# mir-group/pair_allegro

Hardware: AMD Instinct MI355X
Metric: atom_steps_per_sec (higher is better)
Workload: dtype f32-equivalent (f16x2 split on the f16 matrix cores, f32 accumulate); 1 GPU; BASELINE config 4: 1000000-atom bulk Si (50^3 diamond cells), model S (l_max=1, U=32, S=64, 2 layers), r_max 5.0 A + skin 1.0 A, NVE dt=1 fs; grid=1x1x1, rebuilds=4, comm=serial, comm_transport=library/hosted/single-rank gather-scatter

## Files before the change

pair_allegro_amd/csrc/allegro_hip.hip:

```cpp
#include "../../include/allegro_hip.h"

#include <pthread.h>
#include <sched.h>

#include <algorithm>
#include <array>
#include <cmath>
#include <cstdio>
#include <cstdlib>
#include <cstring>
#include <atomic>
#include <condition_variable>
#include <functional>
#include <map>
#include <mutex>
#include <new>
#include <string>
#include <thread>
#include <vector>

#include "engine.h"
#include "generic_engine.h"

using namespace ahip;
// ... 274 lines not shown
    } else if (k == "cutoff_compare") {
      m->cutoff_strict = word("le|lt") == 1;
      m->h_cutsq_dev.clear();
    } else if (k == "edge_schedule") {
      m->opt_edge_schedule = (Model::EdgeSchedule)word(Model::EDGE_SCHEDULE_WORDS);
    } else if (k == "tile_pack") {
      m->opt_tile_pack = (Model::TilePack)word(Model::TILE_PACK_WORDS);
    } else if (k == "dense_centres") {
      m->opt_dense_centres = (Model::DenseCentres)word(Model::DENSE_CENTRES_WORDS);
    } else if (k == "wide_tile") {
      const Model::WideTile o = (Model::WideTile)word(Model::WIDE_TILE_WORDS);
      if (o != m->opt_wide_tile) { m->opt_wide_tile = o; fusedlx_free(*m); }
    } else if (k == "lx64_mlp_width") {
      const Model::Lx64MlpWidth o = (Model::Lx64MlpWidth)word(Model::LX64_MLP_WIDTH_WORDS);
      if (o != m->opt_lx64_mlp_width) { m->opt_lx64_mlp_width = o; fusedlx_free(*m); }
    } else if (k == "timing") {
      m->timing = (v == "1" || v == "on" || v == "true");
    } else throw ArgError("unknown option '" + k + "'");
  });
}

namespace ahip {
namespace {
struct Staging {
  std::mutex mu;
  void *p = nullptr;
  std::map<int, std::array<hipEvent_t, 2>> evs;
  hipEvent_t *ev = nullptr;
  static constexpr size_t BYTES = 8u << 20, HALF = BYTES / 2;
  void *get() {
// ... 1032 lines not shown
```

pair_allegro_amd/csrc/engine.h:

```cpp
#pragma once
#include <hip/hip_runtime.h>

#include <atomic>
#include <map>
#include <stdexcept>
#include <algorithm>
#include <cmath>
#include <cstdlib>
#include <string>
#include <vector>

#include "arith_policy.h"
#include "fused_shapes.h"
#include "model_io.h"
#include "prims.h"

namespace ahip {

struct HipError : std::runtime_error {
  explicit HipError(const std::string &m) : std::runtime_error(m) {}
};
struct ArgError : std::runtime_error {
  explicit ArgError(const std::string &m) : std::runtime_error(m) {}
};
// ... 72 lines not shown

  enum class Path { Auto, Fused, Generic };
  static constexpr const char *PATH_WORDS = "auto|fused|generic";
  enum class Precision { Model, Float64 };
  static constexpr const char *PRECISION_WORDS = "model|float64";
  enum class TilePack { Auto, Separate, Fused };
  static constexpr const char *TILE_PACK_WORDS = "auto|separate|fused";
  enum class EdgeSchedule { Auto, Static, Dynamic };
  static constexpr const char *EDGE_SCHEDULE_WORDS = "auto|static|dynamic";
  enum class DenseCentres { Whole, Split };
  static constexpr const char *DENSE_CENTRES_WORDS = "whole|split";
  enum class WideTile { S64, Auto };
  static constexpr const char *WIDE_TILE_WORDS = "64|auto";
  enum class Lx64MlpWidth { W64, Auto };
  static constexpr const char *LX64_MLP_WIDTH_WORDS = "64|auto";
  Path opt_path = Path::Auto;
  Precision opt_precision = Precision::Model;
  FusedTb opt_fused_tb = FusedTb::Table;
  ArithState arith;
  DevBuf b_chk;
  HostModel hm_fused;
  bool hm_fused_ready = false;
  std::vector<int> active;
  std::vector<int> active_set;
  std::vector<int> active_mapped;
  unsigned char *slot_dev = nullptr;
  const unsigned char *slot_cur = nullptr;
  std::vector<double> rcut_fused_host;
  double *rcut_fused_dev = nullptr;
  long long chunk_edges = 2000000;
  int reserve_wgs = 0;
  bool timing = false;
  TilePack opt_tile_pack = TilePack::Auto;
  EdgeSchedule opt_edge_schedule = EdgeSchedule::Auto;
  DenseCentres opt_dense_centres = DenseCentres::Whole;
  WideTile opt_wide_tile = WideTile::S64;
  Lx64MlpWidth opt_lx64_mlp_width = Lx64MlpWidth::W64;
  bool cutoff_strict = false;

  DeviceWeights<float> wf;
  DeviceWeights<double> wd;
  void *cg_dev = nullptr;
  int ncg_full = 0, ncg_scalar = 0;
  double *rcut_model_dev = nullptr;

  int inum = 0, nall = 0;
  long long nneigh = 0;
  bool have_list = false;
  int max_list_row = -1;
  const int *d_ilist = nullptr, *d_nloff = nullptr, *d_nlj = nullptr;
  DevBuf b_ilist, b_nloff, b_nlj;
  std::vector<int> h_flat_j, h_off32, h_ilist;
// ... 191 lines not shown
```

pair_allegro_amd/csrc/fused.hip:

```cpp
#include <hip/hip_runtime.h>

#include <cmath>
#include <algorithm>
#include <cstdio>
#include <cstdlib>
#include <cstring>
#include <type_traits>

#include "../../include/allegro_hip.h"
#include "engine.h"
#define AHIP_RING 4
#include "fused_common.h"
#include "fused_h.h"
#include "fused_rows.h"
#include "prims.h"

#ifndef AHIP_FUSED_PART
#define AHIP_FUSED_PART 0
#endif
namespace ahip {


[[maybe_unused]] static constexpr int MAX_TILE_SLOTS = 128;
static constexpr int MAXNL = 3;
// ... 15 lines not shown
  const int *maxdeg_sel;
  const float *wbase;
  int wbytes;
  int o_stream;
  int o_tbtab, tb_nk;
  int o_tpl, o_pair, o_out1, o_scale, o_shift;
  int o_res[MAXNL];
  float *scratch;
  long long wg_scratch, wave_scratch;
  double *f, *eatom, *partial;
  long long *prof;
  float *dbg;
  float cp[6];
  int *err;
  double *vatom;
};

template <int NW, int NL = MAXNL, int RT = 2> struct __attribute__((aligned(16))) Lds {
  static constexpr int SLOTS = 16 * NW;
  static constexpr int MAXA = NW == 4 ? 6 : 12;
  float stage[SLOTS * STG_LD];
  float env[NL][MAXA * ENV_LD];
  float denv[MAXA * ENV_LD];
  float tp[NL][5 * 32];
  float park[NW][8 * ROW];
  double eacc[MAXA];
  double virw[NW][6];
  int aoff[2][MAXA + 2];
  float rc[16];
  float scale[16], shift[16];
// ... 124 lines not shown
      acc3 += lds.stage[(sl + 3) * STG_LD + fidx];
    }
    for (; sl < s1; ++sl) acc0 += lds.stage[sl * STG_LD + fidx];
    dst[a * ENV_LD + fidx] = scale * ((acc0 + acc1) + (acc2 + acc3));
  }
}
enum { PH_GEOM = 0, PH_TB, PH_EMB, PH_ENV, PH_TP, PH_MIX, PH_LAT, PH_OUT, PH_BLAT, PH_BMIX, PH_BTP, PH_BENV, PH_BEMB, PH_BTB, PH_FIN, PH_N };
#define PHASE(id) do { if (PROF) { long long _t = clock64(); pacc[id] += _t - tprev; tprev = _t; } } while (0)

template <int AR> struct RingT {
  int act = 1;
  f32x4 f[AR != 0 ? 1 : RING];
  u32x4 b[AR == 0 ? 1 : (AR == 1 ? RINGB : AR == 2 ? RINGB2 : RINGH)];
};
template <int AR, int KT, int NT, bool ACC, int RPI, bool BR = true, class Epi>
__device__ __forceinline__ void lin(__amdgpu_buffer_rsrc_t W, int &wp, const f32x4 (&in)[KT], f32x4 (&out)[NT], int v16, RingT<AR> &ring, Epi epi) {
  if (BR && !ring.act) {
    if constexpr (!ACC) {
#pragma unroll
      for (int t = 0; t < NT; ++t) out[t] = f32x4{0.f, 0.f, 0.f, 0.f};
    }
    return;
  }
  if constexpr (AR == 3) {
    static_assert(KT % 2 == 0, "K-steps are pairs of 16-feature tiles");
    Hop b[1][KT / 2], unused[1][NT / 2];
#pragma unroll
    for (int ks = 0; ks < KT / 2; ++ks) b[0][ks] = split_pair_h(in[2 * ks], in[2 * ks + 1]);
    Epi ep[1] = {epi};
    linear_h<1, KT / 2, NT, ACC, false, (4 * RPI) % RINGH, Epi, true>(W, wp, b, reinterpret_cast<f32x4 (&)[1][NT]>(out), unused, v16, ring.b, ep);
  } else if constexpr (AR != 0) {
    static_assert(KT % 2 == 0, "K-steps are pairs of 16-feature tiles");
    constexpr int NTERM = AR == 1 ? 3 : 2;
    Bop b[KT / 2], unused[NT / 2];
#pragma unroll
    for (int ks = 0; ks < KT / 2; ++ks) b[ks] = split_pair(in[2 * ks], in[2 * ks + 1]);
    linear_b<KT / 2, NT, ACC, false, (2 * NTERM * RPI) % RingB<NTERM>::N, Epi, NTERM>(W, wp, b, out, unused, v16, ring.b, epi);
  } else {
    linear_s<KT, NT, ACC, (4 * RPI) % RING, Epi>(W, wp, in, out, v16, ring.f, epi);
  }
}

template <int RPI, bool BR = true, class Epi>
__device__ __forceinline__ void lin_m3(__amdgpu_buffer_rsrc_t W, int &wp, const f32x4 (&in0)[2], const f32x4 (&in1)[2], const f32x4 (&in2)[2], f32x4 (&out)[3][2], int v16,
                                       RingT<3> &ring, Epi (&epi)[3]) {
  if (BR && !ring.act) {
#pragma unroll
    for (int q = 0; q < 3; ++q) { out[q][0] = f32x4{0.f, 0.f, 0.f, 0.f}; out[q][1] = f32x4{0.f, 0.f, 0.f, 0.f}; }
    return;
  }
  Hop b[3][1], unused[3][1];
  b[0][0] = split_pair_h(in0[0], in0[1]); b[1][0] = split_pair_h(in1[0], in1[1]); b[2][0] = split_pair_h(in2[0], in2[1]);
  linear_h<3, 1, 2, false, false, (4 * RPI) % RINGH, Epi, true>(W, wp, b, out, unused, v16, ring.b, epi);
}
template <class Epi0, class Epi3>
__device__ __forceinline__ void lin_mix(__amdgpu_buffer_rsrc_t W, int &wp, const f32x4 (&in0)[2], const f32x4 (&in1)[2], const f32x4 (&in2)[2], const f32x4 (&in3)[2], f32x4 (&out0)[2],
                                        f32x4 (&out)[3][2], int v16, RingT<3> &ring, Epi0 epi0, Epi3 (&epi)[3]) {
  if (!ring.act) {
    out0[0] = f32x4{0.f, 0.f, 0.f, 0.f}; out0[1] = f32x4{0.f, 0.f, 0.f, 0.f};
#pragma unroll
    for (int q = 0; q < 3; ++q) { out[q][0] = f32x4{0.f, 0.f, 0.f, 0.f}; out[q][1] = f32x4{0.f, 0.f, 0.f, 0.f}; }
    return;
  }
  lin<3, 2, 2, false, 0, false>(W, wp, in0, out0, v16, ring, epi0);
  lin_m3<1, false>(W, wp, in1, in2, in3, out, v16, ring, epi);
}

struct TileIn {
  int a0, a1, e0, e1;
  float rx, ry, rz;
  int eii, jat, tt;
  int eoff;
};
struct TileBounds { int a0, a1, e0, e1; };
typedef const __attribute__((address_space(4))) int *cint_p;
__device__ __forceinline__ TileBounds tile_bounds(const FusedArgs &A, int tile, int ntiles) {
  const int tc = max(min(tile, ntiles - 1), 0);
  const cint_p ta = (cint_p)(unsigned long long)A.tile_a0, te = (cint_p)(unsigned long long)A.tile_e0;
  TileBounds b = {ta[tc], ta[tc + 1], te[tc], te[tc + 1]};
  if (tile >= ntiles) b = TileBounds{0, 0, 0, 0};
// ... 50 lines not shown
    const int pth = (k % 160) / 32;
    if (RT != 2 && k >= (NLT - 1) * 160 + 64) continue;
    lds.tp[k / 160][k % 160] = Wb[A.o_tpl + k] * (pth == 1 ? C_P1 : pth == 4 ? C_P4 : 1.f);
  }
  const int ntiles = *A.ntiles;
  constexpr int NL = NLT;
  double acc_part = 0.0;
  long long pacc[PH_N];
  long long tprev = 0;
  const long long t_clk0 = clock64(), t_wall0 = wall_clock64();
  if (PROF) {
#pragma unroll
    for (int k = 0; k < PH_N; ++k) pacc[k] = 0;
    tprev = clock64();
  }
  float *const pk = lds.park[wave];
  RingT<AR> ring;
  int wp = A.o_stream;
  if constexpr (AR != 0) ring_prime_b(WB, wp, v16, ring.b);
  else ring_prime(WB, wp, v16, ring.f);
  if (tid < MAXA) lds.eacc[tid] = 0.0;
  if (lane < 6) lds.virw[wave][lane] = 0.0;
  if (A.T <= 4 && tid < A.T * A.T) lds.rc[tid] = (float)A.rcut[tid];
  if (tid < A.T) { lds.scale[tid] = Wb[A.o_scale + tid]; lds.shift[tid] = Wb[A.o_shift + tid]; }
  if (tid < 2 * A.NL) lds.res[tid >> 1][tid & 1] = Wb[A.o_res[tid >> 1] + (tid & 1)];
  if constexpr (RT == 2) { if (tid >= 64 && tid < 96) lds.wo1[tid - 64] = Wb[A.o_out1 + tid - 64]; }
  else { if (tid >= 64 && tid < 64 + 16 * RT) lds.wo1v()[tid - 64] = Wb[A.o_out1 + tid - 64]; }

  const int s = wave * 16 + j;
  float *const st = lds.stage + s * STG_LD;
  if (tid == 0) lds.chunk[0] = (int)atomicAdd(A.tile_counter, (unsigned)A.tchunk);
// ... 3 lines not shown

  TileIn nx_;
  tile_fetch(A, tile_bounds(A, cbase, ntiles), s, tid, nx_);
  asm volatile("" : "+v"(nx_.rx), "+v"(nx_.ry), "+v"(nx_.rz), "+v"(nx_.eii), "+v"(nx_.jat), "+v"(nx_.tt), "+v"(nx_.eoff));

  for (;;) {
    const int tile = cbase + ck;
    if (tile >= ntiles) break;
    int claimed = 0;
    if (ck == 0 && tid == 0) {
      unsigned long long tcnt = (unsigned long long)A.tile_counter;
      asm volatile("" : "+v"(tcnt));
      claimed = (int)__hip_atomic_fetch_add((__attribute__((address_space(1))) unsigned int *)tcnt, (unsigned)A.tchunk, __ATOMIC_RELAXED, __HIP_MEMORY_SCOPE_AGENT);
    }
    const int a0 = nx_.a0, a1 = nx_.a1, e0 = nx_.e0, e1 = nx_.e1;
    const int wact = __builtin_amdgcn_readfirstlane(e0 + wave * 16 < e1 ? 1 : 0);
    ring.act = wact;
    const int v16t = wact ? v16 : 0x7ffffff0;
    const int na = a1 - a0;
    par ^= 1;
    int *const aoffp = lds.aoff[par];
    const int e = e0 + s;
    const bool valid = e < e1;
    const float rx = valid ? nx_.rx : 1.f, ry = nx_.ry, rz = nx_.rz;
    const int aloc = valid ? nx_.eii - a0 : 0, jat = nx_.jat, ti = nx_.tt >> 4, tj = nx_.tt & 15;
    if (tid <= na) aoffp[tid] = nx_.eoff - e0;
    const float d = sqrtf(rx * rx + ry * ry + rz * rz);
    const float inv = 1.f / d;
    const float nx = rx * inv, ny = ry * inv, nz = rz * inv;
    const float rc = A.T <= 4 ? lds.rc[ti * A.T + tj] : (float)A.rcut[ti * A.T + tj];
    const float xx = d / rc;
    float fc, dfc_dx;
    cutoff_poly_c(A.p, A.cp, xx, fc, dfc_dx);
    if (!valid) { fc = 0.f; dfc_dx = 0.f; }
// ... 2 lines not shown
    const float PI = 3.14159265358979323846f;
    const float *const envrow = lds.env[0] + aloc * ENV_LD;
    const float *const denvrow = lds.denv + aloc * ENV_LD;
    PHASE(PH_GEOM);

    f32x4 x[4];
    float tb_t = 0.f, tb_invh = 0.f;
    if constexpr (TBT) {
      tb_invh = (float)A.tb_nk / rc;
      const float sft = d * tb_invh;
      const int kq = min((int)sft, A.tb_nk - 1);
      tb_t = sft - (float)kq;
#ifdef ABL_NOTBGATHER
      const int tb_off = (A.o_tbtab + 4 * g) * 4;
#else
      const int tb_off = (A.o_tbtab + ((ti * A.T + tj) * A.tb_nk + kq) * 256 + 4 * g) * 4;
#endif
      const float vm = (valid && xx < 1.f) ? 1.f : 0.f;
#pragma unroll
      for (int t = 0; t < 4; ++t) {
        const f32x4 c0 = bload_w(WB, tb_off + (t * 4 + 0) * 64, 0), c1 = bload_w(WB, tb_off + (t * 4 + 1) * 64, 0);
        const f32x4 c2 = bload_w(WB, tb_off + (t * 4 + 2) * 64, 0), c3 = bload_w(WB, tb_off + (t * 4 + 3) * 64, 0);
        x[t] = (c0 + tb_t * (c1 + tb_t * (c2 + tb_t * c3))) * vm;
        bstore(SB, v16t, (R_Z1TB() + t) * ROW * 4, (c1 + tb_t * (2.f * c2 + (3.f * tb_t) * c3)) * (vm * tb_invh));
      }
    } else {
      f32x4 z[4], z2[4];
      {
        const float *pt = Wb + A.o_pair + (size_t)(ti * A.T + tj) * 64;
#pragma unroll
        for (int t = 0; t < 4; ++t) z[t] = *(const f32x4 *)(pt + 16 * t + 4 * g);
// ... 173 lines not shown
    eps = gsum(eps);
    asm volatile("" : "+v"(eps));

    float bsc = 1.f;
    if constexpr (AR == 3) {
      int bex;
      (void)frexpf(lds.scale[ti] * A.cenv, &bex);
      bex = min(max(bex, -100), 100);
      bsc = ldexpf(1.f, -bex);
      if (g == 0) st[128] = ldexpf(1.f, bex);
    }
    const float deps = valid ? lds.scale[ti] * A.cenv * bsc : 0.f;
    f32x4 dx[4];
    f32x4 dzr[RT];
    if constexpr (RT != 2) {
      const float *wq = lds.wo1v() + 4 * g;
      asm volatile("" : "+v"(wq));
#pragma unroll
      for (int t = 0; t < RT; ++t) wo1[t] = *(const f32x4 *)(wq + 16 * t);
    }
#pragma unroll
    for (int t = 0; t < RT; ++t)
#pragma unroll
      for (int r = 0; r < 4; ++r) dzr[t][r] = deps * wo1[t][r] * dsilu1(zo[t][r]);
    if constexpr (RD == 2) {
      f32x4 dhr[RT];
      lin<AR, RT, RT, false, 1>(WB, wp, dzr, dhr, v16t, ring, EpiNone{});
#pragma unroll
      for (int t = 0; t < RT; ++t)
#pragma unroll
        for (int r = 0; r < 4; ++r) dzr[t][r] = dhr[t][r] * dsilu1(zr[t][r]);
// ... 65 lines not shown
        }
        if constexpr (MD >= 2) {
          if (STGROWS && STG2 && last) {
#pragma unroll
            for (int t = 0; t < 4; ++t) zt1[t] = stg_load(st + 4 * g, t);
          }
        }
        if (kk > 0) {
          if (!(PARKV && last)) {
#pragma unroll
            for (int lm = 0; lm < 4; ++lm) load_rows<2>(SB, RL + OVIN + 2 * lm, Vk[lm], v16t);
          }
        } else load_rows<4>(SB, R_W0(), W0b, v16t);
        __builtin_amdgcn_sched_barrier(0);
        f32x4 dcat[6];
        if constexpr (MD == 1) lin<AR, WT, 6, false, 0>(WB, wp, dh, dcat, v16t, ring, EpiNone{});
        else {
          f32x4 zt0[WT];
          if constexpr (MD == 3) load_rows<WT>(SB, RL + R_OZ(1, WT), zt0, v16t);
          lin<AR, WT, WT, false, 0>(WB, wp, dh, du, v16t, ring, EpiMulRows<WT>{zt1});
          if constexpr (MD == 3) {
            lin<AR, WT, WT, false, 0>(WB, wp, du, dh, v16t, ring, EpiMulRows<WT>{zt0});
            lin<AR, WT, 6, false, 0>(WB, wp, dh, dcat, v16t, ring, EpiNone{});
          } else lin<AR, WT, 6, false, 0>(WB, wp, du, dcat, v16t, ring, EpiNone{});
        }
#pragma unroll
        for (int t = 0; t < 4; ++t) dx[t] += dcat[t];
        dVp[0][0] = dcat[4]; dVp[0][1] = dcat[5];
      }
      if (kk == 0) {
#pragma unroll
        for (int t = 0; t < 2; ++t) {
          Vk[0][t] = W0b[t];
          Vk[1][t] = W0b[2 + t] * Y1; Vk[2][t] = W0b[2 + t] * Y2; Vk[3][t] = W0b[2 + t] * Y3;
        }
      }
      if (PARKV && last && kk > 0) {
#pragma unroll
        for (int lm = 0; lm < 4; ++lm)
#pragma unroll
          for (int t = 0; t < 2; ++t) Vk[lm][t] = park_load(pk, 2 * lm + t, lane);
      }
      f32x4 om1[2];
      load_rows<2>(SB, RL + 2, om1, v16t);
      __builtin_amdgcn_sched_barrier(0);
      PHASE(PH_BLAT);
      if (!last) {
        f32x4 in2[2], o2[2];
        in2[0] = park_load(pk, 0, lane); in2[1] = park_load(pk, 1, lane);
        if constexpr (AR == 3) {
          f32x4 i1[2] = {park_load(pk, 2, lane), park_load(pk, 3, lane)}, i2[2] = {park_load(pk, 4, lane), park_load(pk, 5, lane)},
                i3[2] = {park_load(pk, 6, lane), park_load(pk, 7, lane)};
          f32x4 o3[3][2];
          EpiNone ep[3];
          lin_mix(WB, wp, in2, i1, i2, i3, o2, o3, v16t, ring, EpiNone{}, ep);
          dVp[0][0] += o2[0]; dVp[0][1] += o2[1];
#pragma unroll
          for (int q = 0; q < 3; ++q) { dVp[1 + q][0] = o3[q][0]; dVp[1 + q][1] = o3[q][1]; }
        } else {
          lin<AR, 2, 2, false, 0>(WB, wp, in2, o2, v16t, ring, EpiNone{});
          dVp[0][0] += o2[0]; dVp[0][1] += o2[1];
          in2[0] = park_load(pk, 2, lane); in2[1] = park_load(pk, 3, lane);
          lin<AR, 2, 2, false, 1>(WB, wp, in2, dVp[1], v16t, ring, EpiNone{});
          in2[0] = park_load(pk, 4, lane); in2[1] = park_load(pk, 5, lane);
          lin<AR, 2, 2, false, 2>(WB, wp, in2, dVp[2], v16t, ring, EpiNone{});
          in2[0] = park_load(pk, 6, lane); in2[1] = park_load(pk, 7, lane);
          lin<AR, 2, 2, false, 3>(WB, wp, in2, dVp[3], v16t, ring, EpiNone{});
        }
      }
      __builtin_amdgcn_sched_barrier(0);
// ... 26 lines not shown
          }
          float *sp = st + b;
          *(f32x4 *)(sp) = b0v; *(f32x4 *)(sp + 32) = b1v; *(f32x4 *)(sp + 64) = b2v; *(f32x4 *)(sp + 96) = b3v;
          park_store(pk, 0 + t, a0v, lane);
          park_store(pk, 2 + t, a1v, lane);
          park_store(pk, 4 + t, a2v, lane);
          park_store(pk, 6 + t, a3v, lane);
          __builtin_amdgcn_sched_barrier(0);
        }
        __syncthreads();
        reduce_stage(lds, aoffp, lds.denv, na, A.cenv, tid);
        __syncthreads();
      }
      __builtin_amdgcn_sched_barrier(0);
      PHASE(PH_BTP);
      {
        f32x4 dom[4];
#pragma unroll
        for (int t = 0; t < 2; ++t) {
          const int b = 16 * t + 4 * g;
          const f32x4 d0 = *(const f32x4 *)(denvrow + b), d1 = *(const f32x4 *)(denvrow + 32 + b), d2 = *(const f32x4 *)(denvrow + 64 + b),
                      d3 = *(const f32x4 *)(denvrow + 96 + b);
          dom[t] = d0;
          dom[2 + t] = d1 * Y1 + d2 * Y2 + d3 * Y3;
          const f32x4 p1 = d1 * om1[t], p2 = d2 * om1[t], p3 = d3 * om1[t];
          dY1 += (p1[0] + p1[1]) + (p1[2] + p1[3]); dY2 += (p2[0] + p2[1]) + (p2[2] + p2[3]); dY3 += (p3[0] + p3[1]) + (p3[2] + p3[3]);
          __builtin_amdgcn_sched_barrier(0);
        }
        asm volatile("" : "+v"(dY1), "+v"(dY2), "+v"(dY3));
        if (kk > 0) {
          if (!SAVEZ) load_rows<4>(SB, R_LAYER(kk - 1, MD, WT) + OU, upre, v16t);
          load_rows<WT>(SB, R_LAYER(kk - 1, MD, WT) + OZL, zt, v16t);
        } else {
          if constexpr (!TBT) {
            load_rows<4>(SB, R_U0(), upre, v16t);
            load_rows<4>(SB, R_Z2TB(), zt, v16t);
          } else if constexpr (WT == 4) load_rows<4>(SB, R_Z1TB(), zt, v16t);
          else {
#pragma unroll
            for (int t = 0; t < 4; ++t) zt[t] = bload(SB, v16t, (R_Z1TB() + t) * ROW * 4);
          }
          load_rows<2>(SB, R_W0() + 2, w0h, v16t);
        }
        __builtin_amdgcn_sched_barrier(0);
        lin<AR, 4, 4, true, 0>(WB, wp, dom, dx, v16t, ring, EpiNone{});
      }
      PHASE(PH_BENV);
    }
    tile_fetch(A, nb_, s, tid, nx_);
    int tidc = tid;
    asm volatile("" : "+v"(tidc));
    auto cil_ = __builtin_amdgcn_raw_buffer_load_b64(list_rsrc(A.centre, 8ll * a0, 8 * na), (tidc >> 4) * 8, 0, 0);
    f32x4 zt1b[4];
    if constexpr (!TBT) load_rows<4>(SB, R_Z1TB(), zt1b, v16t);
    __builtin_amdgcn_sched_barrier(0);
    {
      f32x4 dw0[4];
#pragma unroll
      for (int t = 0; t < 2; ++t) {
        const f32x4 d0 = park_load(pk, 0 + t, lane), d1 = park_load(pk, 2 + t, lane), d2 = park_load(pk, 4 + t, lane), d3 = park_load(pk, 6 + t, lane);
// ... 68 lines not shown
          atomicAdd(&A.f[3 * (size_t)jat + 1], -(double)gy);
          atomicAdd(&A.f[3 * (size_t)jat + 2], -(double)gz);
#endif
        }
      }
      float w6[6] = {-rx * gx, -ry * gy, -rz * gz, -0.5f * (rx * gy + ry * gx), -0.5f * (rx * gz + rz * gx), -0.5f * (ry * gz + rz * gy)};
#pragma unroll
      for (int c = 0; c < 6; ++c) w6[c] = valid ? w6[c] : 0.f;
#pragma unroll
      for (int c = 0; c < 6; ++c) {
#pragma unroll
        for (int off = 8; off > 0; off >>= 1) w6[c] += __shfl_xor(w6[c], off, 64);
      }
      if (lane < 6) {
        const float mine = lane == 0 ? w6[0] : lane == 1 ? w6[1] : lane == 2 ? w6[2] : lane == 3 ? w6[3] : lane == 4 ? w6[4] : w6[5];
        lds.virw[wave][lane] += (double)mine;
      }
      if constexpr (VA) vatom_scatter(A.vatom, jat, g, valid, rx, ry, rz, gx, gy, gz);
    }
    int tidf = tid;
    asm volatile("" : "+v"(tidf));
    const int caf = tidf >> 4;
    __syncthreads();
    const int2 cil = make_int2((int)cil_[0], (int)cil_[1]);
    {
      const int col = tidf & 3, part = (tidf >> 2) & 3;
      float sum = 0.f;
      if (caf < na)
        for (int sl = aoffp[caf] + part; sl < aoffp[caf + 1]; sl += 4) sum += lds.stage[sl * STG_LD + col];
      sum += __shfl_xor(sum, 4, 64);
      sum += __shfl_xor(sum, 8, 64);
// ... 53 lines not shown
}
#endif
#if AHIP_FUSED_PART == 3
void fused_launch_f16_rd2(int nw, int md, int grid, hipStream_t s, const FusedArgs &A) {
  dispatch<Choices<4, 8>, Choices<1, 2, 3>, Choices<1, 3, 2>, Choices<VAR_VA, VAR_PLAIN>>([&](auto nw, auto nl, auto md, auto var) {
    hipLaunchKernelGGL((k_fused<nw, false, 3, true, nl, md, var == VAR_VA, 2>), dim3(grid), dim3(nw * 64), 0, s, A);
  }, nw, A.NL, md, fused_variant(A.vatom, false));
}
#endif
#if AHIP_FUSED_PART == 2
void fused_launch_f16(int nw, bool prof, int md, int grid, hipStream_t s, const FusedArgs &A) {
#ifdef AHIP_ASM_ONLY
#ifndef AHIP_ASM_NW
#define AHIP_ASM_NW 4
#endif
  hipLaunchKernelGGL((k_fused<AHIP_ASM_NW, false, 3, true, 2, 2>), dim3(grid), dim3(AHIP_ASM_NW * 64), 0, s, A);
#else
  dispatch<Choices<4, 8>, Choices<1, 2, 3>, Choices<1, 3, 2>, Variants>([&](auto nw, auto nl, auto md, auto var) {
    if constexpr (var != VAR_PROF || md == 2) hipLaunchKernelGGL((k_fused<nw, var == VAR_PROF, 3, true, nl, md, var == VAR_VA>), dim3(grid), dim3(nw * 64), 0, s, A);
  }, nw, A.NL, md, fused_variant(A.vatom, prof && md == 2));
#endif
}
#endif
#if AHIP_FUSED_PART == 1
void fused_launch_bf16(int nw, bool prof, int arith, bool tbt, int grid, hipStream_t s, const FusedArgs &A) {
  dispatch<Choices<4, 8>, Choices<1, 2>, Choices<1, 0>, Choices<1, 2, 3>, Variants>([&](auto nw, auto b3, auto tb, auto nl, auto var) {
    hipLaunchKernelGGL((k_fused<nw, var == VAR_PROF, b3, tb != 0, nl, 2, var == VAR_VA>), dim3(grid), dim3(nw * 64), 0, s, A);
  }, nw, arith, tbt, A.NL, fused_variant(A.vatom, prof));
}
#endif

// ... 178 lines not shown
      if (why) *why = "an atom has " + std::to_string(m.last_max_deg) + " edges (> 128 per tile)";
      return false;
    }
    nw = m.last_max_deg <= 64 ? 4 : 8;
    if (st.force_nw == 8 || (st.force_nw == 4 && m.last_max_deg <= 64)) nw = st.force_nw;
  } else if (st.force_nw == 8) nw = 8;
  else if (m.max_list_row >= 0 && m.max_list_row <= 64) nw = 4;
  const int *maxdeg_sel = nw == 0 ? m.d_maxdeg : nullptr;
  m.arith.last = st.arith;
  hipStream_t s = a.stream;
  const int tile_slots = nw == 8 ? 128 : 64, maxa = nw == 8 ? Lds<8>::MAXA : Lds<4>::MAXA;
  static_assert(Lds<4>::MAXA == FUSED_TILE_MAXA && FUSED_TILE_SLOTS == 64, "allegro_hip.hip requests the 4-wave tile shape from the edge build");
  FusedArgs A = st.args;
  fused_tile_args(m, st.tiles, a, A, tile_slots, maxa, maxdeg_sel, nw == 4);
  A.maxdeg_sel = maxdeg_sel;
  const long long nedges_est = fused_nedges_estimate(m);
  const int grid4 = std::max(1, st.ncu * 2 - m.reserve_wgs), grid8 = std::max(1, st.ncu - m.reserve_wgs);
  const int grid = nw == 8 ? grid8 : grid4;
  if (nw == 0) AHIP_CHECK(hipMemsetAsync(st.tiles.partial.p, 0, (size_t)grid * 7 * sizeof(double), s));
  {
    StageTimer tm(m, "model_fused", s);
    if (st.dbg_on) {
      st.dbg.reserve((size_t)std::max<long long>(m.nedges, 1) * 8 * sizeof(float));
      AHIP_CHECK(hipMemsetAsync(st.dbg.p, 0, (size_t)m.nedges * 8 * sizeof(float), s));
      A.dbg = st.dbg.as<float>();
    }
    if (st.prof_on || st.clk_on) {
      AHIP_CHECK(hipMemsetAsync(st.prof.p, 0, (64 + 4 * (size_t)grid) * sizeof(long long), s));
      A.prof = st.prof.as<long long>();
    }
// ... 224 lines not shown
```

pair_allegro_amd/csrc/fused_h.h:

```cpp
#pragma once
#include <cstring>

#include "fused_common.h"

namespace ahip {

typedef _Float16 f16x2 __attribute__((ext_vector_type(2)));
typedef _Float16 f16x8 __attribute__((ext_vector_type(8)));
typedef float f32x2 __attribute__((ext_vector_type(2)));
struct Hop { u32x4 hi, lo; };
static constexpr float H_LO_SCALE = 2048.f, H_LO_INV = 1.f / 2048.f;
static constexpr int RINGH = 8;
constexpr int lin_frags_h(int KT, int NT) { return 4 * (NT / 2) * (KT / 2); }

__device__ __forceinline__ f32x4 mfma_h(u32x4 a, u32x4 b, f32x4 c) {
  return __builtin_amdgcn_mfma_f32_16x16x32_f16(__builtin_bit_cast(f16x8, a), __builtin_bit_cast(f16x8, b), c, 0, 0, 0);
}
__device__ __forceinline__ void split2_h(float v0, float v1, unsigned &hi, unsigned &lo) {
  const f32x2 v = {v0, v1};
  const f16x2 h = __builtin_convertvector(v, f16x2);
  const f32x2 r = (v - __builtin_convertvector(h, f32x2)) * H_LO_SCALE;
  const f16x2 l = __builtin_convertvector(r, f16x2);
  hi = __builtin_bit_cast(unsigned, h);
  lo = __builtin_bit_cast(unsigned, l);
// ... 8 lines not shown
  return b;
}

__device__ __forceinline__ void ring_prime_h(__amdgpu_buffer_rsrc_t W, int wp, int v16, u32x4 (&ring)[RINGH]) {
  int wo = wp * 4;
  pin_s(wo);
#pragma unroll
  for (int j = 0; j < RINGH; ++j) ring[j] = __builtin_bit_cast(u32x4, bload_w(W, v16 + (j & 3) * 1024, wo + (j >> 2) * 4096));
}

template <class E> __device__ __forceinline__ auto epi_apply2(E &e, int ot, int r, f32x2 v, int) -> decltype(e.apply2(ot, r, v)) { return e.apply2(ot, r, v); }
template <class E> __device__ __forceinline__ f32x2 epi_apply2(E &e, int ot, int r, f32x2 v, long) { return f32x2{e.apply(ot, r, v[0]), e.apply(ot, r + 1, v[1])}; }

template <int G, int KS, int NT, bool ACC, bool SPLIT, int RP, class Epi, bool LATE_OK = false>
__device__ __forceinline__ void linear_h(__amdgpu_buffer_rsrc_t W, int &wp, const Hop (&in)[G][KS], f32x4 (&out)[G][NT], Hop (&outb)[G][NT / 2],
                                         int v16, u32x4 (&ring)[RINGH], Epi (&epi)[G]) {
  static_assert(NT % 2 == 0, "output tiles are processed in pairs");
  constexpr int RB = RINGH, NF = 4, NP = NT / 2, NSTEP = NP * KS, NS = NF * NSTEP;
  constexpr int MF = 6 * G;
#ifndef AHIP_LATE_STEPS
#define AHIP_LATE_STEPS 2
#endif
  constexpr bool LATE = LATE_OK && NSTEP <= AHIP_LATE_STEPS;
  f32x4 ah[G][2], ac[G][2], prev[G][2];
  int wo = (wp + RB * 256) * 4;
  pin_s(wo);
#pragma unroll
  for (int s = 0; s < NSTEP; ++s) {
    const int p = s / KS, ks = s % KS;
    if (ks == 0) {
#pragma unroll
      for (int g = 0; g < G; ++g)
#pragma unroll
        for (int hh = 0; hh < 2; ++hh) {
          ah[g][hh] = ACC ? out[g][2 * p + hh] : f32x4{0.f, 0.f, 0.f, 0.f};
          ac[g][hh] = f32x4{0.f, 0.f, 0.f, 0.f};
        }
    }
    u32x4 a[NF];
#pragma unroll
    for (int i = 0; i < NF; ++i) a[i] = ring[(RP + NF * s + i) % RB];
    if (!LATE) {
#pragma unroll
      for (int q = 0; q < NF; ++q) {
        const int i = LATE_OK ? (q + 2) % NF : q;
        ring[(RP + NF * s + i) % RB] = __builtin_bit_cast(u32x4, bload_w(W, v16 + i * 1024, wo));
      }
    }
    if (!LATE) {
      wo += NF * 1024;
      pin_s(wo);
    }
#pragma unroll
    for (int m = 0; m < 3; ++m) {
#pragma unroll
      for (int hh = 0; hh < 2; ++hh) {
#pragma unroll
        for (int g = 0; g < G; ++g) {
          if (m == 0) ac[g][hh] = mfma_h(a[2 + hh], in[g][ks].hi, ac[g][hh]);
          else if (m == 1) ac[g][hh] = mfma_h(a[hh], in[g][ks].lo, ac[g][hh]);
          else ah[g][hh] = mfma_h(a[hh], in[g][ks].hi, ah[g][hh]);
          if (LATE && g == G - 1 && m != 1) {
            const int i = m == 0 ? 2 + hh : hh;
            ring[(RP + NF * s + i) % RB] = __builtin_bit_cast(u32x4, bload_w(W, v16 + i * 1024, wo));
          }
          if (p > 0) {
            const int idx = ks * MF + (m * 2 + hh) * G + g, tot = KS * MF, NE = 4 * G;
            const int e0 = (idx * NE + tot - 1) / tot, e1 = ((idx + 1) * NE + tot - 1) / tot;
#pragma unroll
            for (int e = 0; e < NE; ++e)
              if (e >= e0 && e < e1) {
                const int eg = e / 4, th = (e % 4) / 2, r = 2 * (e % 2), ot = 2 * (p - 1) + th;
                const f32x2 y = epi_apply2(epi[eg], ot, r, f32x2{prev[eg][th][r], prev[eg][th][r + 1]}, 0);
                out[eg][ot][r] = y[0]; out[eg][ot][r + 1] = y[1];
                if (e % 4 == 3) {
                  epi[eg].flush(2 * (p - 1));
                  if (SPLIT) outb[eg][p - 1] = split_pair_h(out[eg][2 * (p - 1)], out[eg][2 * (p - 1) + 1]);
                }
              }
// ... 72 lines not shown
```

Baseline: 29.26 million atom-steps/s.

## Add centre-level environment backward for small-tile four-wave fused kernel

Adds an env_backward option; in the AR==3, NW=4 fused kernel, tiles with at most three centres compute the environment-backward linear once per centre on one wave and share the per-centre products through LDS. Other waves skip that matmul and advance the weight stream by jumping ring prefetch offsets. This removes redundant per-edge MFMA work in the backward environment step. In exchange it adds a workgroup barrier and extra LDS traffic. It also reworks the weight-ring prefetch addressing, which is delicate to get right.

```diff
diff --git a/pair_allegro_amd/csrc/allegro_hip.hip b/pair_allegro_amd/csrc/allegro_hip.hip
--- a/pair_allegro_amd/csrc/allegro_hip.hip
+++ b/pair_allegro_amd/csrc/allegro_hip.hip
@@ -312,6 +312,8 @@
     } else if (k == "lx64_mlp_width") {
       const Model::Lx64MlpWidth o = (Model::Lx64MlpWidth)word(Model::LX64_MLP_WIDTH_WORDS);
       if (o != m->opt_lx64_mlp_width) { m->opt_lx64_mlp_width = o; fusedlx_free(*m); }
+    } else if (k == "env_backward") {
+      m->opt_env_backward = (Model::EnvBackward)word(Model::ENV_BACKWARD_WORDS);
     } else if (k == "timing") {
       m->timing = (v == "1" || v == "on" || v == "true");
     } else throw ArgError("unknown option '" + k + "'");
diff --git a/pair_allegro_amd/csrc/engine.h b/pair_allegro_amd/csrc/engine.h
--- a/pair_allegro_amd/csrc/engine.h
+++ b/pair_allegro_amd/csrc/engine.h
@@ -110,6 +110,8 @@
   static constexpr const char *WIDE_TILE_WORDS = "64|auto";
   enum class Lx64MlpWidth { W64, Auto };
   static constexpr const char *LX64_MLP_WIDTH_WORDS = "64|auto";
+  enum class EnvBackward { Auto, Centre, Edge };
+  static constexpr const char *ENV_BACKWARD_WORDS = "auto|centre|edge";
   Path opt_path = Path::Auto;
   Precision opt_precision = Precision::Model;
   FusedTb opt_fused_tb = FusedTb::Table;
@@ -132,6 +134,7 @@
   DenseCentres opt_dense_centres = DenseCentres::Whole;
   WideTile opt_wide_tile = WideTile::S64;
   Lx64MlpWidth opt_lx64_mlp_width = Lx64MlpWidth::W64;
+  EnvBackward opt_env_backward = EnvBackward::Auto;
   bool cutoff_strict = false;
 
   DeviceWeights<float> wf;
diff --git a/pair_allegro_amd/csrc/fused.hip b/pair_allegro_amd/csrc/fused.hip
--- a/pair_allegro_amd/csrc/fused.hip
+++ b/pair_allegro_amd/csrc/fused.hip
@@ -53,6 +53,7 @@
   float cp[6];
   int *err;
   double *vatom;
+  int env_bwd;
 };
 
 template <int NW, int NL = MAXNL, int RT = 2> struct __attribute__((aligned(16))) Lds {
@@ -207,7 +208,7 @@
   u32x4 b[AR == 0 ? 1 : (AR == 1 ? RINGB : AR == 2 ? RINGB2 : RINGH)];
 };
 template <int AR, int KT, int NT, bool ACC, int RPI, bool BR = true, class Epi>
-__device__ __forceinline__ void lin(__amdgpu_buffer_rsrc_t W, int &wp, const f32x4 (&in)[KT], f32x4 (&out)[NT], int v16, RingT<AR> &ring, Epi epi) {
+__device__ __forceinline__ void lin(__amdgpu_buffer_rsrc_t W, int &wp, const f32x4 (&in)[KT], f32x4 (&out)[NT], int v16, RingT<AR> &ring, Epi epi, int jump = 0) {
   if (BR && !ring.act) {
     if constexpr (!ACC) {
 #pragma unroll
@@ -221,7 +222,7 @@
 #pragma unroll
     for (int ks = 0; ks < KT / 2; ++ks) b[0][ks] = split_pair_h(in[2 * ks], in[2 * ks + 1]);
     Epi ep[1] = {epi};
-    linear_h<1, KT / 2, NT, ACC, false, (4 * RPI) % RINGH, Epi, true>(W, wp, b, reinterpret_cast<f32x4 (&)[1][NT]>(out), unused, v16, ring.b, ep);
+    linear_h<1, KT / 2, NT, ACC, false, (4 * RPI) % RINGH, Epi, true>(W, wp, b, reinterpret_cast<f32x4 (&)[1][NT]>(out), unused, v16, ring.b, ep, jump);
   } else if constexpr (AR != 0) {
     static_assert(KT % 2 == 0, "K-steps are pairs of 16-feature tiles");
     constexpr int NTERM = AR == 1 ? 3 : 2;
@@ -236,7 +237,7 @@
 
 template <int RPI, bool BR = true, class Epi>
 __device__ __forceinline__ void lin_m3(__amdgpu_buffer_rsrc_t W, int &wp, const f32x4 (&in0)[2], const f32x4 (&in1)[2], const f32x4 (&in2)[2], f32x4 (&out)[3][2], int v16,
-                                       RingT<3> &ring, Epi (&epi)[3]) {
+                                       RingT<3> &ring, Epi (&epi)[3], int jump = 0) {
   if (BR && !ring.act) {
 #pragma unroll
     for (int q = 0; q < 3; ++q) { out[q][0] = f32x4{0.f, 0.f, 0.f, 0.f}; out[q][1] = f32x4{0.f, 0.f, 0.f, 0.f}; }
@@ -244,19 +245,19 @@
   }
   Hop b[3][1], unused[3][1];
   b[0][0] = split_pair_h(in0[0], in0[1]); b[1][0] = split_pair_h(in1[0], in1[1]); b[2][0] = split_pair_h(in2[0], in2[1]);
-  linear_h<3, 1, 2, false, false, (4 * RPI) % RINGH, Epi, true>(W, wp, b, out, unused, v16, ring.b, epi);
+  linear_h<3, 1, 2, false, false, (4 * RPI) % RINGH, Epi, true>(W, wp, b, out, unused, v16, ring.b, epi, jump);
 }
 template <class Epi0, class Epi3>
 __device__ __forceinline__ void lin_mix(__amdgpu_buffer_rsrc_t W, int &wp, const f32x4 (&in0)[2], const f32x4 (&in1)[2], const f32x4 (&in2)[2], const f32x4 (&in3)[2], f32x4 (&out0)[2],
-                                        f32x4 (&out)[3][2], int v16, RingT<3> &ring, Epi0 epi0, Epi3 (&epi)[3]) {
+                                        f32x4 (&out)[3][2], int v16, RingT<3> &ring, Epi0 epi0, Epi3 (&epi)[3], int jump = 0) {
   if (!ring.act) {
     out0[0] = f32x4{0.f, 0.f, 0.f, 0.f}; out0[1] = f32x4{0.f, 0.f, 0.f, 0.f};
 #pragma unroll
     for (int q = 0; q < 3; ++q) { out[q][0] = f32x4{0.f, 0.f, 0.f, 0.f}; out[q][1] = f32x4{0.f, 0.f, 0.f, 0.f}; }
     return;
   }
-  lin<3, 2, 2, false, 0, false>(W, wp, in0, out0, v16, ring, epi0);
-  lin_m3<1, false>(W, wp, in1, in2, in3, out, v16, ring, epi);
+  lin<3, 2, 2, false, 0, false>(W, wp, in0, out0, v16, ring, epi0, jump);
+  lin_m3<1, false>(W, wp, in1, in2, in3, out, v16, ring, epi, jump);
 }
 
 struct TileIn {
@@ -337,7 +338,7 @@
     for (int k = 0; k < PH_N; ++k) pacc[k] = 0;
     tprev = clock64();
   }
-  float *const pk = lds.park[wave];
+  float *const pk0 = lds.park[wave];
   RingT<AR> ring;
   int wp = A.o_stream;
   if constexpr (AR != 0) ring_prime_b(WB, wp, v16, ring.b);
@@ -371,10 +372,23 @@
       claimed = (int)__hip_atomic_fetch_add((__attribute__((address_space(1))) unsigned int *)tcnt, (unsigned)A.tchunk, __ATOMIC_RELAXED, __HIP_MEMORY_SCOPE_AGENT);
     }
     const int a0 = nx_.a0, a1 = nx_.a1, e0 = nx_.e0, e1 = nx_.e1;
-    const int wact = __builtin_amdgcn_readfirstlane(e0 + wave * 16 < e1 ? 1 : 0);
+    constexpr bool CEN = AR == 3 && NW == 4;
+    int tq = tid, lq_ = lane, wvq = wave;
+    if constexpr (CEN) {
+      asm volatile("" : "+v"(tq));
+      wvq = __builtin_amdgcn_readfirstlane(tq >> 6);
+      lq_ = tq & 63;
+    }
+    float *const pk = CEN ? lds.park[wvq] : pk0;
+    const int wact = __builtin_amdgcn_readfirstlane(e0 + wvq * 16 < e1 ? 1 : 0);
     ring.act = wact;
     const int v16t = wact ? v16 : 0x7ffffff0;
     const int na = a1 - a0;
+    int cen = 0;
+    if constexpr (CEN) {
+      if (A.env_bwd != 2 && na <= 3) cen = !wact ? 3 : wvq == 0 ? 1 : 2;
+    }
+    const int cjump = cen == 2 ? 16 * 1024 : 0;
     par ^= 1;
     int *const aoffp = lds.aoff[par];
     const int e = e0 + s;
@@ -407,7 +421,7 @@
 #ifdef ABL_NOTBGATHER
       const int tb_off = (A.o_tbtab + 4 * g) * 4;
 #else
-      const int tb_off = (A.o_tbtab + ((ti * A.T + tj) * A.tb_nk + kq) * 256 + 4 * g) * 4;
+      const int tb_off = (A.o_tbtab + ((ti * A.T + tj) * A.tb_nk + kq) * 256 + 4 * (lq_ >> 4)) * 4;
 #endif
       const float vm = (valid && xx < 1.f) ? 1.f : 0.f;
 #pragma unroll
@@ -611,7 +625,7 @@
     f32x4 dx[4];
     f32x4 dzr[RT];
     if constexpr (RT != 2) {
-      const float *wq = lds.wo1v() + 4 * g;
+      const float *wq = lds.wo1v() + 4 * (lq_ >> 4);
       asm volatile("" : "+v"(wq));
 #pragma unroll
       for (int t = 0; t < RT; ++t) wo1[t] = *(const f32x4 *)(wq + 16 * t);
@@ -707,15 +721,16 @@
         } else load_rows<4>(SB, R_W0(), W0b, v16t);
         __builtin_amdgcn_sched_barrier(0);
         f32x4 dcat[6];
-        if constexpr (MD == 1) lin<AR, WT, 6, false, 0>(WB, wp, dh, dcat, v16t, ring, EpiNone{});
+        const int dj = last ? cjump : 0;
+        if constexpr (MD == 1) lin<AR, WT, 6, false, 0>(WB, wp, dh, dcat, v16t, ring, EpiNone{}, dj);
         else {
           f32x4 zt0[WT];
           if constexpr (MD == 3) load_rows<WT>(SB, RL + R_OZ(1, WT), zt0, v16t);
           lin<AR, WT, WT, false, 0>(WB, wp, dh, du, v16t, ring, EpiMulRows<WT>{zt1});
           if constexpr (MD == 3) {
             lin<AR, WT, WT, false, 0>(WB, wp, du, dh, v16t, ring, EpiMulRows<WT>{zt0});
-            lin<AR, WT, 6, false, 0>(WB, wp, dh, dcat, v16t, ring, EpiNone{});
-          } else lin<AR, WT, 6, false, 0>(WB, wp, du, dcat, v16t, ring, EpiNone{});
+            lin<AR, WT, 6, false, 0>(WB, wp, dh, dcat, v16t, ring, EpiNone{}, dj);
+          } else lin<AR, WT, 6, false, 0>(WB, wp, du, dcat, v16t, ring, EpiNone{}, dj);
         }
 #pragma unroll
         for (int t = 0; t < 4; ++t) dx[t] += dcat[t];
@@ -746,7 +761,7 @@
                 i3[2] = {park_load(pk, 6, lane), park_load(pk, 7, lane)};
           f32x4 o3[3][2];
           EpiNone ep[3];
-          lin_mix(WB, wp, in2, i1, i2, i3, o2, o3, v16t, ring, EpiNone{}, ep);
+          lin_mix(WB, wp, in2, i1, i2, i3, o2, o3, v16t, ring, EpiNone{}, ep, cjump);
           dVp[0][0] += o2[0]; dVp[0][1] += o2[1];
 #pragma unroll
           for (int q = 0; q < 3; ++q) { dVp[1 + q][0] = o3[q][0]; dVp[1 + q][1] = o3[q][1]; }
@@ -803,7 +818,23 @@
       }
       __builtin_amdgcn_sched_barrier(0);
       PHASE(PH_BTP);
-      {
+      auto next_rows = [&]() __attribute__((always_inline)) {
+        if (kk > 0) {
+          if (!SAVEZ) load_rows<4>(SB, R_LAYER(kk - 1, MD, WT) + OU, upre, v16t);
+          load_rows<WT>(SB, R_LAYER(kk - 1, MD, WT) + OZL, zt, v16t);
+        } else {
+          if constexpr (!TBT) {
+            load_rows<4>(SB, R_U0(), upre, v16t);
+            load_rows<4>(SB, R_Z2TB(), zt, v16t);
+          } else if constexpr (WT == 4) load_rows<4>(SB, R_Z1TB(), zt, v16t);
+          else {
+#pragma unroll
+            for (int t = 0; t < 4; ++t) zt[t] = bload(SB, v16t, (R_Z1TB() + t) * ROW * 4);
+          }
+          load_rows<2>(SB, R_W0() + 2, w0h, v16t);
+        }
+      };
+      if constexpr (!CEN) {
         f32x4 dom[4];
 #pragma unroll
         for (int t = 0; t < 2; ++t) {
@@ -817,22 +848,72 @@
           __builtin_amdgcn_sched_barrier(0);
         }
         asm volatile("" : "+v"(dY1), "+v"(dY2), "+v"(dY3));
-        if (kk > 0) {
-          if (!SAVEZ) load_rows<4>(SB, R_LAYER(kk - 1, MD, WT) + OU, upre, v16t);
-          load_rows<WT>(SB, R_LAYER(kk - 1, MD, WT) + OZL, zt, v16t);
-        } else {
-          if constexpr (!TBT) {
-            load_rows<4>(SB, R_U0(), upre, v16t);
-            load_rows<4>(SB, R_Z2TB(), zt, v16t);
-          } else if constexpr (WT == 4) load_rows<4>(SB, R_Z1TB(), zt, v16t);
-          else {
-#pragma unroll
-            for (int t = 0; t < 4; ++t) zt[t] = bload(SB, v16t, (R_Z1TB() + t) * ROW * 4);
-          }
-          load_rows<2>(SB, R_W0() + 2, w0h, v16t);
-        }
+        next_rows();
         __builtin_amdgcn_sched_barrier(0);
         lin<AR, 4, 4, true, 0>(WB, wp, dom, dx, v16t, ring, EpiNone{});
+      } else {
+        float *const pm = lds.env[0] + kk * (MAXA * ENV_LD);
+        static_assert(2 * ENV_LD >= 4 * 64 && 3 * 2 * ENV_LD <= Lds<NW>::MAXA * ENV_LD, "the per-centre products of three centres fit a layer's environment rows");
+        auto dy_sums = [&]() __attribute__((always_inline)) {
+#pragma unroll
+          for (int t = 0; t < 2; ++t) {
+            const int b = 16 * t + 4 * g;
+            const f32x4 p1 = *(const f32x4 *)(denvrow + 32 + b) * om1[t], p2 = *(const f32x4 *)(denvrow + 64 + b) * om1[t], p3 = *(const f32x4 *)(denvrow + 96 + b) * om1[t];
+            dY1 += (p1[0] + p1[1]) + (p1[2] + p1[3]); dY2 += (p2[0] + p2[1]) + (p2[2] + p2[3]); dY3 += (p3[0] + p3[1]) + (p3[2] + p3[3]);
+          }
+          asm volatile("" : "+v"(dY1), "+v"(dY2), "+v"(dY3));
+        };
+        next_rows();
+        if (cen != 1) dy_sums();
+        if (cen < 2) {
+          const float *dr = denvrow + 4 * g;
+          float m0 = 1.f, m1 = Y1, m2 = Y2, m3 = Y3;
+          int pcol = 0;
+          if (cen == 1) {
+            int lq = lane;
+            asm volatile("" : "+v"(lq));
+            const int c = (lq >> 2) & 3, q = lq & 3, gq = lq >> 4;
+            const bool on = c < na;
+            dr = lds.denv + c * ENV_LD + 4 * gq;
+            m0 = on && q == 0 ? 1.f : 0.f; m1 = on && q == 1 ? 1.f : 0.f; m2 = on && q == 2 ? 1.f : 0.f; m3 = on && q == 3 ? 1.f : 0.f;
+            pcol = c < 3 ? c * (2 * ENV_LD) + 64 * q + 4 * gq : -1;
+#pragma unroll
+            for (int t = 0; t < 4; ++t) { *(f32x4 *)(st + 16 * t + 4 * g) = dx[t]; dx[t] = f32x4{0.f, 0.f, 0.f, 0.f}; }
+          }
+          f32x4 dom[4];
+#pragma unroll
+          for (int t = 0; t < 2; ++t) {
+            const f32x4 d0 = *(const f32x4 *)(dr + 16 * t), d1 = *(const f32x4 *)(dr + 32 + 16 * t), d2 = *(const f32x4 *)(dr + 64 + 16 * t), d3 = *(const f32x4 *)(dr + 96 + 16 * t);
+            dom[t] = d0 * m0;
+            dom[2 + t] = d1 * m1 + d2 * m2 + d3 * m3;
+          }
+          __builtin_amdgcn_sched_barrier(0);
+          lin<AR, 4, 4, true, 0>(WB, wp, dom, dx, v16t, ring, EpiNone{});
+          if (cen == 1) {
+            if (pcol >= 0) {
+#pragma unroll
+              for (int t = 0; t < 4; ++t) *(f32x4 *)(pm + pcol + 16 * t) = dx[t];
+            }
+#pragma unroll
+            for (int t = 0; t < 4; ++t) dx[t] = *(const f32x4 *)(st + 16 * t + 4 * g);
+          }
+        } else if (cen == 2) {
+          wp += lin_frags_h(4, 4) * 256;
+          pin_s(wp);
+        }
+        if (cen) {
+          __syncthreads();
+          if (cen == 1) dy_sums();
+          if (cen != 3) {
+            const float *pr = pm + 2 * (envrow - lds.env[0]) + 4 * g;
+#pragma unroll
+            for (int t = 0; t < 4; ++t) {
+              const f32x4 p0 = *(const f32x4 *)(pr + 16 * t), p1 = *(const f32x4 *)(pr + 64 + 16 * t), p2 = *(const f32x4 *)(pr + 128 + 16 * t),
+                          p3 = *(const f32x4 *)(pr + 192 + 16 * t);
+              dx[t] += p0 + Y1 * p1 + Y2 * p2 + Y3 * p3;
+            }
+          }
+        }
       }
       PHASE(PH_BENV);
     }
@@ -931,7 +1012,7 @@
       }
       if (lane < 6) {
         const float mine = lane == 0 ? w6[0] : lane == 1 ? w6[1] : lane == 2 ? w6[2] : lane == 3 ? w6[3] : lane == 4 ? w6[4] : w6[5];
-        lds.virw[wave][lane] += (double)mine;
+        lds.virw[wvq][lq_] += (double)mine;
       }
       if constexpr (VA) vatom_scatter(A.vatom, jat, g, valid, rx, ry, rz, gx, gy, gz);
     }
@@ -1015,7 +1096,22 @@
 #ifndef AHIP_ASM_NW
 #define AHIP_ASM_NW 4
 #endif
-  hipLaunchKernelGGL((k_fused<AHIP_ASM_NW, false, 3, true, 2, 2>), dim3(grid), dim3(AHIP_ASM_NW * 64), 0, s, A);
+#ifndef AHIP_ASM_NL
+#define AHIP_ASM_NL 2
+#endif
+#ifndef AHIP_ASM_MD
+#define AHIP_ASM_MD 2
+#endif
+#ifndef AHIP_ASM_VA
+#define AHIP_ASM_VA false
+#endif
+#ifndef AHIP_ASM_WT
+#define AHIP_ASM_WT 4
+#endif
+#ifndef AHIP_ASM_RT
+#define AHIP_ASM_RT 2
+#endif
+  hipLaunchKernelGGL((k_fused<AHIP_ASM_NW, false, 3, true, AHIP_ASM_NL, AHIP_ASM_MD, AHIP_ASM_VA, 1, AHIP_ASM_WT, AHIP_ASM_RT>), dim3(grid), dim3(AHIP_ASM_NW * 64), 0, s, A);
 #else
   dispatch<Choices<4, 8>, Choices<1, 2, 3>, Choices<1, 3, 2>, Variants>([&](auto nw, auto nl, auto md, auto var) {
     if constexpr (var != VAR_PROF || md == 2) hipLaunchKernelGGL((k_fused<nw, var == VAR_PROF, 3, true, nl, md, var == VAR_VA>), dim3(grid), dim3(nw * 64), 0, s, A);
@@ -1224,6 +1320,7 @@
   FusedArgs A = st.args;
   fused_tile_args(m, st.tiles, a, A, tile_slots, maxa, maxdeg_sel, nw == 4);
   A.maxdeg_sel = maxdeg_sel;
+  A.env_bwd = (int)m.opt_env_backward;
   const long long nedges_est = fused_nedges_estimate(m);
   const int grid4 = std::max(1, st.ncu * 2 - m.reserve_wgs), grid8 = std::max(1, st.ncu - m.reserve_wgs);
   const int grid = nw == 8 ? grid8 : grid4;
diff --git a/pair_allegro_amd/csrc/fused_h.h b/pair_allegro_amd/csrc/fused_h.h
--- a/pair_allegro_amd/csrc/fused_h.h
+++ b/pair_allegro_amd/csrc/fused_h.h
@@ -46,7 +46,7 @@
 
 template <int G, int KS, int NT, bool ACC, bool SPLIT, int RP, class Epi, bool LATE_OK = false>
 __device__ __forceinline__ void linear_h(__amdgpu_buffer_rsrc_t W, int &wp, const Hop (&in)[G][KS], f32x4 (&out)[G][NT], Hop (&outb)[G][NT / 2],
-                                         int v16, u32x4 (&ring)[RINGH], Epi (&epi)[G]) {
+                                         int v16, u32x4 (&ring)[RINGH], Epi (&epi)[G], int jump = 0) {
   static_assert(NT % 2 == 0, "output tiles are processed in pairs");
   constexpr int RB = RINGH, NF = 4, NP = NT / 2, NSTEP = NP * KS, NS = NF * NSTEP;
   constexpr int MF = 6 * G;
@@ -72,11 +72,12 @@
     u32x4 a[NF];
 #pragma unroll
     for (int i = 0; i < NF; ++i) a[i] = ring[(RP + NF * s + i) % RB];
+    const int wr = s >= NSTEP - 2 ? wo + jump : wo;
     if (!LATE) {
 #pragma unroll
       for (int q = 0; q < NF; ++q) {
         const int i = LATE_OK ? (q + 2) % NF : q;
-        ring[(RP + NF * s + i) % RB] = __builtin_bit_cast(u32x4, bload_w(W, v16 + i * 1024, wo));
+        ring[(RP + NF * s + i) % RB] = __builtin_bit_cast(u32x4, bload_w(W, v16 + i * 1024, wr));
       }
     }
     if (!LATE) {
@@ -94,7 +95,7 @@
           else ah[g][hh] = mfma_h(a[hh], in[g][ks].hi, ah[g][hh]);
           if (LATE && g == G - 1 && m != 1) {
             const int i = m == 0 ? 2 + hh : hh;
-            ring[(RP + NF * s + i) % RB] = __builtin_bit_cast(u32x4, bload_w(W, v16 + i * 1024, wo));
+            ring[(RP + NF * s + i) % RB] = __builtin_bit_cast(u32x4, bload_w(W, v16 + i * 1024, wr));
           }
           if (p > 0) {
             const int idx = ks * MF + (m * 2 + hh) * G + g, tot = KS * MF, NE = 4 * G;
```

After: 29.58 million atom-steps/s, median of 6. 1.01x the previous value.
